# MrTornado24/FENeRF

Hardware: NVIDIA H100
Metric: rendered faces/sec at 128px x 24 samples/ray (higher is better)
Workload: dtype f16 operands / f32 accumulate (wgmma) + f32 refinement

## Files before the change

fenerf_b200/csrc/mapping.cu:

```cuda
#include "common.cuh"

namespace fn {

namespace {

constexpr int kMaxB = 32;
constexpr unsigned kFull = 0xffffffffu;

struct HiddenArgs {
    const float* w[4];
    const float* b[4];
    const float* z;
    float* h_out;
    int B, z_dim;
};

constexpr int kChunkB = 8;

__global__ void __launch_bounds__(256) mapping_hidden_kernel(HiddenArgs a) {
    extern __shared__ __align__(16) float xs[];
    const int warp = threadIdx.x >> 5, lane = threadIdx.x & 31;
    const int B = a.B;
    float* x0 = xs;
    float* x1 = xs + (size_t)B * 512;
    for (int i = threadIdx.x; i < B * a.z_dim; i += blockDim.x) x0[(i / a.z_dim) * 512 + (i % a.z_dim)] = a.z[i];
    __syncthreads();
    int K = a.z_dim;
    for (int layer = 0; layer < 4; ++layer) {
        const float* W = a.w[layer];
        const float* bias = a.b[layer];
        const float* xin = (layer & 1) ? x1 : x0;
        float* xout = (layer & 1) ? x0 : x1;
#pragma unroll 1
        for (int og = 0; og < 4; ++og) {
        float4 wreg[8][4];
#pragma unroll
        for (int o = 0; o < 8; ++o)
#pragma unroll
            for (int it = 0; it < 4; ++it) {
                const int k = lane * 4 + it * 128;
                wreg[o][it] = k < K ? __ldg(reinterpret_cast<const float4*>(W + (size_t)(warp * 32 + og * 8 + o) * K + k)) : make_float4(0.f, 0.f, 0.f, 0.f);
            }
#pragma unroll
        for (int o = 0; o < 8; ++o) {
            const int f = warp * 32 + og * 8 + o;
            for (int b0 = 0; b0 < B; b0 += kChunkB) {
                float acc[kChunkB];
#pragma unroll
                for (int b = 0; b < kChunkB; ++b) acc[b] = 0.f;
#pragma unroll
                for (int it = 0; it < 4; ++it) {
                    const int k = lane * 4 + it * 128;
                    if (k < K) {
                        const float4 wv = wreg[o][it];
#pragma unroll
                        for (int b = 0; b < kChunkB; ++b)
                            if (b0 + b < B) {
                                const float4 xv = *reinterpret_cast<const float4*>(xin + (b0 + b) * 512 + k);
                                acc[b] = fmaf(wv.x, xv.x, fmaf(wv.y, xv.y, fmaf(wv.z, xv.z, fmaf(wv.w, xv.w, acc[b]))));
                            }
                    }
                }
#pragma unroll
                for (int b = 0; b < kChunkB; ++b)
                    if (b0 + b < B) {
                        float v = acc[b];
#pragma unroll
                        for (int off = 16; off > 0; off >>= 1) v += __shfl_xor_sync(kFull, v, off);
                        v += bias[f];
                        v = v > 0.f ? v : 0.2f * v;
                        if (lane == 0) {
                            if (layer == 3) a.h_out[(b0 + b) * 256 + f] = v;
                            else xout[(b0 + b) * 512 + f] = v;
                        }
                    }
            }
        }
        }
        __syncthreads();
        K = 256;
    }
}

struct OutArgs {
    const float* w;
    const float* b;
    const float* h;
    const float* avg_f;
    const float* avg_p;
    float* film;
    int B, n_layers, layer0, n_film_total;
    float psi;
};

__global__ void __launch_bounds__(256) mapping_out_kernel(OutArgs a) {
    extern __shared__ __align__(16) float hs[];
    const int B = a.B;
    for (int i = threadIdx.x; i < B * 256; i += blockDim.x) hs[i] = a.h[i];
    __syncthreads();
    const int warp = threadIdx.x >> 5, lane = threadIdx.x & 31;
    const int half = a.n_layers * 256, n_out = 2 * half;
    for (int r = blockIdx.x * 8 + warp; r < n_out; r += gridDim.x * 8) {
        const float4 w0 = *reinterpret_cast<const float4*>(a.w + (size_t)r * 256 + lane * 8);
        const float4 w1 = *reinterpret_cast<const float4*>(a.w + (size_t)r * 256 + lane * 8 + 4);
        const float bias = a.b[r];
        const bool is_freq = r < half;
        const int j = is_freq ? r : r - half, l = j >> 8, f = j & 255;
        for (int b = 0; b < B; ++b) {
            const float4 x0 = *reinterpret_cast<const float4*>(hs + b * 256 + lane * 8);
            const float4 x1 = *reinterpret_cast<const float4*>(hs + b * 256 + lane * 8 + 4);
            float v = fmaf(w0.x, x0.x, fmaf(w0.y, x0.y, fmaf(w0.z, x0.z, w0.w * x0.w)));
            v = fmaf(w1.x, x1.x, fmaf(w1.y, x1.y, fmaf(w1.z, x1.z, fmaf(w1.w, x1.w, v))));
#pragma unroll
            for (int off = 16; off > 0; off >>= 1) v += __shfl_xor_sync(kFull, v, off);
            if (lane == 0) {
                v += bias;
                if (a.avg_f) {
                    const float avg = is_freq ? a.avg_f[j] : a.avg_p[j];
                    v = __fadd_rn(avg, __fmul_rn(a.psi, __fsub_rn(v, avg)));
                }
                if (is_freq) v = __fadd_rn(__fmul_rn(v, 15.f), 30.f);
                a.film[(((size_t)b * a.n_film_total + a.layer0 + l) * 2 + (is_freq ? 0 : 1)) * 256 + f] = v;
            }
        }
    }
}

}

int mapping_film(const float* const* w, const float* const* b, const float* z, int B, int z_dim, int n_layers, int layer0,
                 int n_film_total, const float* avg_f, const float* avg_p, float psi, float* h_scratch, float* film,
                 cudaStream_t st) {
    FN_REQUIRE(z_dim >= 4 && z_dim <= 512 && z_dim % 4 == 0, "z_dim %d unsupported (multiple of 4, <= 512)", z_dim);
    for (int b0 = 0; b0 < B; b0 += kMaxB) {
        const int nb = (B - b0) < kMaxB ? (B - b0) : kMaxB;
        HiddenArgs ha;
        for (int i = 0; i < 4; ++i) { ha.w[i] = w[i]; ha.b[i] = b[i]; }
        ha.z = z + (size_t)b0 * z_dim; ha.h_out = h_scratch; ha.B = nb; ha.z_dim = z_dim;
        const size_t smem_h = (size_t)2 * nb * 512 * sizeof(float);
        if (int e = launch<mapping_hidden_kernel>("mapping_hidden_kernel", 1, 256, smem_h, st, ha)) return e;
        OutArgs oa;
        oa.w = w[4]; oa.b = b[4]; oa.h = h_scratch; oa.avg_f = avg_f; oa.avg_p = avg_p;
        oa.film = film + (size_t)b0 * n_film_total * 512; oa.B = nb; oa.n_layers = n_layers; oa.layer0 = layer0;
        oa.n_film_total = n_film_total; oa.psi = psi;
        const int rows = n_layers * 512;
        int blocks = (rows + 7) / 8;
        if (blocks > num_sms() * 2) blocks = num_sms() * 2;
        mapping_out_kernel<<<blocks, 256, (size_t)nb * 256 * sizeof(float), st>>>(oa);
        FN_LAUNCH_OK("mapping_out_kernel");
    }
    return 0;
}

}
```

Baseline: 661.4.

## Split mapping hidden MLP across an 8-CTA cluster with DSMEM broadcast

The mapping network's hidden layers ran on a single CTA. They now run on a thread-block cluster of 8 CTAs. Each warp owns 4 output features per layer and preloads all four layers' weights into registers up front. Each layer's activations are broadcast to every CTA's shared memory through distributed shared memory, with cluster.sync between layers. This spreads the serial mapping MLP across more SMs, at the cost of cluster-wide barriers, remote shared-memory writes and heavy register use.

```diff
diff --git a/fenerf_b200/csrc/mapping.cu b/fenerf_b200/csrc/mapping.cu
--- a/fenerf_b200/csrc/mapping.cu
+++ b/fenerf_b200/csrc/mapping.cu
@@ -1,8 +1,11 @@
 #include "common.cuh"
+#include <cooperative_groups.h>
 
 namespace fn {
 
 namespace {
+
+namespace cg = cooperative_groups;
 
 constexpr int kMaxB = 32;
 constexpr unsigned kFull = 0xffffffffu;
@@ -15,35 +18,43 @@
     int B, z_dim;
 };
 
+constexpr int kCtas = 8;
+constexpr int kFeat = 256 / (kCtas * 8);
 constexpr int kChunkB = 8;
 
-__global__ void __launch_bounds__(256) mapping_hidden_kernel(HiddenArgs a) {
+__global__ void __cluster_dims__(kCtas, 1, 1) __launch_bounds__(256, 1) mapping_hidden_kernel(HiddenArgs a) {
     extern __shared__ __align__(16) float xs[];
+    cg::cluster_group cluster = cg::this_cluster();
     const int warp = threadIdx.x >> 5, lane = threadIdx.x & 31;
     const int B = a.B;
+    const int f0 = ((int)cluster.block_rank() * 8 + warp) * kFeat;
+    float4 wreg[4][kFeat][4];
+#pragma unroll
+    for (int layer = 0; layer < 4; ++layer) {
+        const int K = layer == 0 ? a.z_dim : 256;
+#pragma unroll
+        for (int o = 0; o < kFeat; ++o)
+#pragma unroll
+            for (int it = 0; it < 4; ++it) {
+                const int k = lane * 4 + it * 128;
+                wreg[layer][o][it] = k < K ? __ldg(reinterpret_cast<const float4*>(a.w[layer] + (size_t)(f0 + o) * K + k))
+                                           : make_float4(0.f, 0.f, 0.f, 0.f);
+            }
+    }
     float* x0 = xs;
     float* x1 = xs + (size_t)B * 512;
     for (int i = threadIdx.x; i < B * a.z_dim; i += blockDim.x) x0[(i / a.z_dim) * 512 + (i % a.z_dim)] = a.z[i];
-    __syncthreads();
-    int K = a.z_dim;
+    cluster.sync();
+#pragma unroll
     for (int layer = 0; layer < 4; ++layer) {
-        const float* W = a.w[layer];
-        const float* bias = a.b[layer];
+        const int K = layer == 0 ? a.z_dim : 256;
         const float* xin = (layer & 1) ? x1 : x0;
         float* xout = (layer & 1) ? x0 : x1;
-#pragma unroll 1
-        for (int og = 0; og < 4; ++og) {
-        float4 wreg[8][4];
+        float* dst = cluster.map_shared_rank(xout, lane % kCtas);
 #pragma unroll
-        for (int o = 0; o < 8; ++o)
-#pragma unroll
-            for (int it = 0; it < 4; ++it) {
-                const int k = lane * 4 + it * 128;
-                wreg[o][it] = k < K ? __ldg(reinterpret_cast<const float4*>(W + (size_t)(warp * 32 + og * 8 + o) * K + k)) : make_float4(0.f, 0.f, 0.f, 0.f);
-            }
-#pragma unroll
-        for (int o = 0; o < 8; ++o) {
-            const int f = warp * 32 + og * 8 + o;
+        for (int o = 0; o < kFeat; ++o) {
+            const int f = f0 + o;
+            const float bias = __ldg(a.b[layer] + f);
             for (int b0 = 0; b0 < B; b0 += kChunkB) {
                 float acc[kChunkB];
 #pragma unroll
@@ -52,7 +63,7 @@
                 for (int it = 0; it < 4; ++it) {
                     const int k = lane * 4 + it * 128;
                     if (k < K) {
-                        const float4 wv = wreg[o][it];
+                        const float4 wv = wreg[layer][o][it];
 #pragma unroll
                         for (int b = 0; b < kChunkB; ++b)
                             if (b0 + b < B) {
@@ -67,18 +78,17 @@
                         float v = acc[b];
 #pragma unroll
                         for (int off = 16; off > 0; off >>= 1) v += __shfl_xor_sync(kFull, v, off);
-                        v += bias[f];
+                        v += bias;
                         v = v > 0.f ? v : 0.2f * v;
-                        if (lane == 0) {
-                            if (layer == 3) a.h_out[(b0 + b) * 256 + f] = v;
-                            else xout[(b0 + b) * 512 + f] = v;
+                        if (layer == 3) {
+                            if (lane == 0) a.h_out[(b0 + b) * 256 + f] = v;
+                        } else if (lane < kCtas) {
+                            dst[(b0 + b) * 512 + f] = v;
                         }
                     }
             }
         }
-        }
-        __syncthreads();
-        K = 256;
+        if (layer < 3) cluster.sync();
     }
 }
 
@@ -138,7 +148,7 @@
         for (int i = 0; i < 4; ++i) { ha.w[i] = w[i]; ha.b[i] = b[i]; }
         ha.z = z + (size_t)b0 * z_dim; ha.h_out = h_scratch; ha.B = nb; ha.z_dim = z_dim;
         const size_t smem_h = (size_t)2 * nb * 512 * sizeof(float);
-        if (int e = launch<mapping_hidden_kernel>("mapping_hidden_kernel", 1, 256, smem_h, st, ha)) return e;
+        if (int e = launch<mapping_hidden_kernel>("mapping_hidden_kernel", kCtas, 256, smem_h, st, ha)) return e;
         OutArgs oa;
         oa.w = w[4]; oa.b = b[4]; oa.h = h_scratch; oa.avg_f = avg_f; oa.avg_p = avg_p;
         oa.film = film + (size_t)b0 * n_film_total * 512; oa.B = nb; oa.n_layers = n_layers; oa.layer0 = layer0;
```

Measured after the change: 671.4, median of 6. 1.02x the previous value.
